# finleygou/GS-MARL

Measured on AMD Instinct MI355X. Metric: agent-steps/sec, coop-navigation 24 agents × 8192 envs, at 1/2/4/8 MI355X, higher is better.
Workload: dtype f32; 1 GPU; cooperative_navigation 24 agents x 8192 envs per GPU (24 goals, 24 obstacles; BASELINE headline / configs[4] shard); scenario=navigation, n_agents=24, n_envs_per_gpu=8192, global_envs=8192, episode_length=100, parallelism=env-sharded x1 (no data-path collective)

## Files before the change

gs-marl_amd/csrc/gsm_seg_kernels.hip:

```cpp
#include <type_traits>

#include "gsm_device.h"

namespace gsm {

template <typename T>
__device__ __forceinline__ T seg_scan(T v, int m) {
#pragma unroll
    for (int o = 1; o < kWave; o <<= 1) {
        const T u = __shfl_up(v, o);
        if (m >= o) v += u;
    }
    return v;
}

__device__ __forceinline__ int row_entity(int m, int N) { return m < N ? m : N + m; }

template <int kN, int kNo>
constexpr int envs_per_wave() {
    return kN > 0 ? ((kWave / (kN + kNo)) > kMaxSegEnvsPerWave ? kMaxSegEnvsPerWave : kWave / (kN + kNo))
                  : 0;
}

template <int kN, int kNo>
// ... 321 lines not shown
    }
    const uint32_t wb_lo = __builtin_amdgcn_readfirstlane((uint32_t)env_off);
    const uint32_t wb_hi = __builtin_amdgcn_readfirstlane((uint32_t)((uint64_t)env_off >> 32));
    const int64_t wbase = (int64_t)(((uint64_t)wb_hi << 32) | wb_lo);
    uint32_t o = (uint32_t)(env_off - wbase) + (uint32_t)(incl - c + (m >= N ? N : 0));
    const uint32_t goal_at = (uint32_t)(env_off - wbase) + (uint32_t)(a_total + m);
    if (!L.live || wbase >= out.cap) return;

    const float2 pm = s_pos[row_entity(m, N)];
    const uint32_t cap = (uint32_t)(out.cap - wbase);
    char *src = (char *)(out.index + wbase), *dst = (char *)(out.index + out.cap + wbase);
    char *attr = (char *)(out.attr + wbase);
    const int32_t g0 = (int32_t)(eb * E);
    const int32_t gs = g0 + row_entity(m, N);
    const uint64_t agent_bits = N >= 64 ? ~0ull : ((1ull << N) - 1);
    auto walk = [&](auto chk) {
        constexpr bool kChecked = decltype(chk)::value;
        auto put = [&](uint32_t at, int32_t a, int32_t b, float d) {
            if (!kChecked || at < cap) {
                const uint32_t byte = at << 2;
                *(int32_t *)(src + byte) = a;
                *(int32_t *)(dst + byte) = b;
                *(float *)(attr + byte) = d;
            }
        };
        auto edge_to = [&](int j, int32_t col) {
            const float2 q = s_pos[j];
            const float dx = pm.x - q.x, dy = pm.y - q.y;
            put(o++, gs, col, __builtin_amdgcn_sqrtf(dx * dx + dy * dy));
        };
        if constexpr (kG == 1 && kN > 0 && kN <= 32 && kN + kNo > 32) {
            const uint32_t gshift = L.agent ? 1u : 0u;
            if (L.agent) {
                const float2 q = s_pos[N + m];
                const float dx = pm.x - q.x, dy = pm.y - q.y;
                put(o + (uint32_t)__popcll(mask & agent_bits), gs, g0 + N + m,
                    __builtin_amdgcn_sqrtf(dx * dx + dy * dy));
            }
            uint64_t w = mask;
            while (w) {
                const int j = __builtin_ctzll(w);
                w &= w - 1;
                const bool ob = j >= kN;
                const int ent = ob ? kN + j : j;
                const float2 q = s_pos[ent];
                const float dx = pm.x - q.x, dy = pm.y - q.y;
                put(o + (ob ? gshift : 0u), gs, g0 + ent, __builtin_amdgcn_sqrtf(dx * dx + dy * dy));
                ++o;
            }
        } else if constexpr (kN > 0 && kN <= 32 && kNo <= 32) {
            uint32_t lo = (uint32_t)(mask & agent_bits), hi = (uint32_t)(mask >> kN);
            while (lo) {
                const int j = __builtin_ctz(lo);
                lo &= lo - 1;
                edge_to(j, g0 + j);
            }
            if (L.agent) edge_to(N + m, g0 + N + m);
            while (hi) {
                const int j = __builtin_ctz(hi);
                hi &= hi - 1;
                edge_to(2 * N + j, g0 + 2 * N + j);
            }
        } else {
            uint64_t lo = mask & agent_bits, hi = mask & ~agent_bits;
            while (lo) {
                const int j = __builtin_ctzll(lo);
                lo &= lo - 1;
                edge_to(j, g0 + j);
            }
            if (L.agent) edge_to(N + m, g0 + N + m);
            while (hi) {
                const int j = __builtin_ctzll(hi);
                hi &= hi - 1;
                edge_to(N + j, g0 + N + j);
            }
        }
        if (L.agent) {
            const float2 g = s_pos[N + m];
            const float dx = pm.x - g.x, dy = pm.y - g.y;
            put(goal_at, g0 + N + m, gs, __builtin_amdgcn_sqrtf(dx * dx + dy * dy));
        }
    };
    if (checked) walk(std::true_type{});
    else walk(std::false_type{});
}

template <int kN, int kNo>
__device__ __forceinline__ int stage_rows(const Lane &L, uint32_t *s_scr, int scr_cap, uint64_t mask, int incl) {
    constexpr int N = kN;
    static_assert(N <= 31 && kNo <= 32, "agent and obstacle column bits in one word each");
    const int m = L.m;
    const uint64_t mk = L.live ? mask : 0ull;
    const uint32_t lo = (uint32_t)mk & ((1u << N) - 1u), hi = (uint32_t)(mk >> N);
    const int c = __popc(lo) + __popc(hi) + (L.agent ? 1 : 0);
    const int a_total = __builtin_amdgcn_readlane(incl, N - 1);
    const int total = __builtin_amdgcn_readlane(incl, 63) + N;
    if (total > scr_cap) return -1;
    uint32_t *at = s_scr + (incl - c + (m >= N ? N : 0));
    const uint32_t src = (uint32_t)row_entity(m, N);
    for (uint32_t w = lo; w; w &= w - 1) *at++ = src | ((uint32_t)__builtin_ctz(w) << 8);
    if (L.agent) {
        *at++ = src | ((uint32_t)(N + m) << 8);
        s_scr[a_total + m] = (uint32_t)(N + m) | ((uint32_t)m << 8);
    }
    for (uint32_t w = hi; w; w &= w - 1) *at++ = src | ((uint32_t)(2 * N + __builtin_ctz(w)) << 8);
    wave_sync();
    return total;
}
template <int kN, int kNo>
__device__ __forceinline__ int stage_rows(const Lane &L, uint32_t *s_scr, int scr_cap, uint64_t mask) {
    const uint64_t mk = L.live ? mask : 0ull;
    const uint32_t lo = (uint32_t)mk & ((1u << kN) - 1u), hi = (uint32_t)(mk >> kN);
    const int c = __popc(lo) + __popc(hi) + (L.agent ? 1 : 0);
    return stage_rows<kN, kNo>(L, s_scr, scr_cap, mask, wave_scan(c));
}
template <int kN, int kNo>
__device__ __forceinline__ void write_staged(const Lane &L, const float2 *s_pos, const uint32_t *s_scr, int total,
                                             int64_t env_off, const EdgeSink &out) {
    constexpr int E = 2 * kN + kNo;
    const int64_t eb = L.b;
    const int32_t g0 = (int32_t)(eb * E);
    if (out.cap < ((int64_t)1 << 29)) {
        const uint32_t wb = (uint32_t)env_off, cap4 = (uint32_t)out.cap * 4u;
        char *const isrc = (char *)out.index, *const attr = (char *)out.attr;
        for (int e = L.lane; e < total; e += kWave) {
            const uint32_t w = s_scr[e];
            const uint32_t a = w & 0xffu, b = w >> 8;
            const float2 pa = s_pos[a], pb = s_pos[b];
            const float dx = pa.x - pb.x, dy = pa.y - pb.y;
            uint32_t byte = (wb + (uint32_t)e) << 2;
            asm("" : "+v"(byte));
            *(int32_t *)(isrc + byte) = g0 + (int32_t)a;
            *(int32_t *)(isrc + (byte + cap4)) = g0 + (int32_t)b;
            *(float *)(attr + byte) = __builtin_amdgcn_sqrtf(dx * dx + dy * dy);
        }
        return;
    }
    const uint32_t wb_lo = __builtin_amdgcn_readfirstlane((uint32_t)env_off);
    const uint32_t wb_hi = __builtin_amdgcn_readfirstlane((uint32_t)((uint64_t)env_off >> 32));
    const int64_t wbase = (int64_t)(((uint64_t)wb_hi << 32) | wb_lo);
    char *isrc = (char *)(out.index + wbase), *idst = (char *)(out.index + out.cap + wbase);
    char *attr = (char *)(out.attr + wbase);
    for (int e = L.lane; e < total; e += kWave) {
        const uint32_t w = s_scr[e];
        const uint32_t a = w & 0xffu, b = w >> 8;
        const float2 pa = s_pos[a], pb = s_pos[b];
        const float dx = pa.x - pb.x, dy = pa.y - pb.y;
        uint32_t byte = (uint32_t)e << 2;
        asm("" : "+v"(byte));
        *(int32_t *)(isrc + byte) = g0 + (int32_t)a;
        *(int32_t *)(idst + byte) = g0 + (int32_t)b;
        *(float *)(attr + byte) = __builtin_amdgcn_sqrtf(dx * dx + dy * dy);
    }
}

struct BlockPrefix {
    int cnt_k, acc;
};
__device__ __forceinline__ BlockPrefix block_prefix_loads(const int32_t *block_sum, const int32_t *edge_count,
                                                          int B, int G, const void *any16) {
    BlockPrefix r{0, 0};
    const int lane = threadIdx.x & 63, tid = threadIdx.x;
    const int first = blockIdx.x * kWavesPerBlock * G;
    const int nblk = min(kWavesPerBlock * G, B - first);
    const int ck = edge_count[first + min(lane, nblk - 1)];
    r.cnt_k = lane < nblk ? ck : 0;
    const int nb = (int)blockIdx.x, n4 = nb >> 2, nb4 = n4 << 2;
    const int4 *bs4 = n4 > 0 ? (const int4 *)block_sum : (const int4 *)any16;
    const int kc = n4 > 0 ? n4 - 1 : 0;
    const int4 q0 = bs4[min(tid, kc)], q1 = bs4[min(tid + kBlock, kc)];
    const int tl = block_sum[min(nb4 + tid, max(nb - 1, 0))];
    r.acc = (tid < n4 ? q0.x + q0.y + q0.z + q0.w : 0) + (tid + kBlock < n4 ? q1.x + q1.y + q1.z + q1.w : 0) +
            (tid < nb - nb4 ? tl : 0);
    for (int k = tid + 2 * kBlock; k < n4; k += kBlock) {
        const int4 q = bs4[k];
        r.acc += q.x + q.y + q.z + q.w;
    }
    return r;
}

template <int kN, int kNo, int kG>
__device__ __forceinline__ void block_emit(const DevParams &p, const Shape<kN, kNo> &s, const Lane &L,
                                           const float2 *s_pos, uint64_t mask, BlockPrefix pre, int *s_red,
                                           int64_t *edge_ptr, const EdgeSink &out, uint32_t *s_scr,
                                           int scr_cap) {
    const int first = blockIdx.x * kWavesPerBlock * s.G;
    constexpr bool kStaged = kG == 1 && kN > 0 && kN <= 31 && kNo <= 32;
    int staged = -1;
    if constexpr (kStaged) {
        if (L.b < p.B) staged = stage_rows<kN, kNo>(L, s_scr, scr_cap, mask);
    }
    const int acc = wave_total(pre.acc);
    const int incl_k = wave_scan(pre.cnt_k);
    if (L.lane == 0) s_red[L.wave] = acc;
    __syncthreads();
    int64_t base = 0;
    for (int q = 0; q < kWavesPerBlock; ++q) base += s_red[q];
    int my_cnt, before;
    if constexpr (kG == 1) {
        my_cnt = __builtin_amdgcn_readlane(pre.cnt_k, L.wave);
        before = __builtin_amdgcn_readlane(incl_k, L.wave) - my_cnt;
    } else {
        const int kk = L.live ? L.b - first : 0;
        my_cnt = __shfl(pre.cnt_k, kk);
        before = __shfl(incl_k, kk) - my_cnt;
    }
    const int64_t env_off = base + before;
    if (L.live && L.m == 0) {
        edge_ptr[L.b] = env_off;
        if (L.b == p.B - 1) edge_ptr[p.B] = env_off + my_cnt;
    }
    if constexpr (kStaged) {
        if (staged >= 0 && env_off + staged <= out.cap) {
            write_staged<kN, kNo>(L, s_pos, s_scr, staged, env_off, out);
            return;
        }
    }
    emit_rows<kN, kNo, kG>(s, L, s_pos, mask, env_off, out, env_off + my_cnt > out.cap);
}

struct SegIn {
    float2 x0, x1, v, u;
    uint64_t cand_prev, oo;
    int t, ep;
    float2 acc;
    float4 araw;
};

template <int kN, int kNo, int kFmt, bool kLag>
__device__ __forceinline__ SegIn seg_load(const DevParams &p, const Shape<kN, kNo> &s, const Lane &L) {
    static_assert(kN > 0 && kFmt >= 0, "compile-time shape and action format");
    constexpr int N = kN, E = 2 * kN + kNo, M = kN + kNo;
    SegIn in;
    const int64_t eb = L.b < p.B ? L.b : p.B - 1;
    const uint32_t lane = (uint32_t)L.lane;
    const uint32_t ma = lane < (uint32_t)N ? lane : N - 1, mm = lane < (uint32_t)M ? lane : M - 1;
    const float2 *pos_b = p.pos + eb * E;
    in.x0 = pos_b[lane < (uint32_t)E ? lane : E - 1];
    in.x1 = E > kWave ? pos_b[lane + kWave < (uint32_t)E ? lane + kWave : E - 1] : make_float2(0.0f, 0.0f);
    in.t = p.step_count[eb];
    in.ep = p.episode[eb];
    in.acc = p.ep_acc[eb];
    in.v = p.vel[eb * N + ma];
    const bool step = p.mode == kModeStep;
    const int64_t ai = eb * N + ma;
    if constexpr (kFmt == 0) {
        const float *q = (step ? (const float *)p.actions : p.node_feat) + ai * 5;
        in.araw = make_float4(q[1], q[2], q[3], q[4]);
    } else if constexpr (kFmt == 1) {
        const int32_t *q = step ? (const int32_t *)p.actions : (const int32_t *)p.node_feat;
        in.araw = make_float4(__int_as_float(q[ai]), 0.0f, 0.0f, 0.0f);
    } else {
        const float2 *q = step ? (const float2 *)p.actions : (const float2 *)p.node_feat;
        const float2 a = q[ai];
        in.araw = make_float4(a.x, a.y, 0.0f, 0.0f);
    }
    in.cand_prev = p.contact_mask[eb * N + ma];
    in.oo = p.row_mask[eb * M + mm];
    return in;
}

template <int kN, int kNo, int kFmt, bool kLag>
__device__ __forceinline__ void seg_load_finish(const DevParams &p, const Lane &L, SegIn &in) {
    const bool step = p.mode == kModeStep;
    const float4 a = in.araw;
    float ux, uy;
    if constexpr (kFmt == 0) {
        ux = a.x - a.y;
        uy = a.z - a.w;
    } else if constexpr (kFmt == 1) {
        const int k = __float_as_int(a.x);
        ux = (float)(k == 1) - (float)(k == 2);
        uy = (float)(k == 3) - (float)(k == 4);
    } else {
        ux = a.x;
        uy = a.y;
    }
    const bool ag_step = L.agent && step;
    in.u = ag_step ? make_float2(ux * p.sens, uy * p.sens) : make_float2(0.0f, 0.0f);
    in.cand_prev = ag_step ? in.cand_prev : 0ull;
    if (!L.agent) in.v = make_float2(0.0f, 0.0f);
    in.oo = (L.live && (kLag || L.m >= kN) && step) ? in.oo : 0ull;
    if (L.b >= p.B) {
        in.t = in.ep = 0;
        in.acc = make_float2(0.0f, 0.0f);
    }
}

template <int kN, int kNo, int kFmt, bool kLag>
__device__ __forceinline__ int seg_env(const DevParams &p, const Shape<kN, kNo> &s, const Lane &L,
                                       unsigned char *wave_lds, const SegIn &in, int64_t wid,
                                       BlockPrefix lag_pre, int *s_lag) {
    constexpr int kG = envs_per_wave<kN, kNo>();
    const int N = s.N, E = s.E, M = s.M, G = s.G;
    const int segc = L.seg < G ? L.seg : G - 1;
    float2 *s_pos = (float2 *)wave_lds + segc * E;
    float *s_nf = (float *)((float2 *)wave_lds + G * E);
    const int m = L.m;
    const bool obst = L.live && m >= N;
    const bool wave_live = kG == 1 ? L.b < p.B : true;
    const int64_t eb = kG == 1 ? (wave_live ? L.b : 0) : (L.live ? L.b : 0);
    const uint32_t um = (uint32_t)m;

    SegIn inf = in;
    if constexpr (kG == 1) seg_load_finish<kN, kNo, kFmt, kLag>(p, L, inf);
    int t = inf.t, ep = inf.ep;
// ... 596 lines not shown
            obs_sweep<kN, kNo, 1, kFused>(late_params(), s, L, s_pos, s_nf, pm2, true, 0ull, row2, cand2, cc2,
                                          coinc2, &Fn2, unext);
            if (reset) {
                pm = pm2;
                row = row2;
                cand = cand2;
                coinc = coinc2;
                Fn = Fn2;
            }
            if (!L.live) row = 0;
            scan = wave_scan(__popcll(row) + (L.agent ? 1 : 0));
            scan_tot = __builtin_amdgcn_readlane(scan, 63);
        }
        GSM_ACC(p, L.b, 15, tr0);
        const bool relaid = reset;
        if constexpr (kFused) {
            if (L.agent) s_force[m] = Fn;
        }

        KernargParams &q = late_params();
        const bool any_statics = (!kPlain && q.nf_full) || __any(relaid);
        if constexpr (kSlots) {
            if (L.live) {
                float *nf = q.ro.nf + k * q.ro.nf_s + eb * E * 7;
                if (L.agent) {
                    const float2 g = s_pos[N + m];
                    store_row(nf + m * 7, v, pm, make_float2(g.x - pm.x, g.y - pm.y), 0.0f);
                    if (any_statics)
                        store_row(nf + (N + m) * 7, make_float2(0.0f, 0.0f), g, make_float2(0.0f, 0.0f), 1.0f);
                } else if (any_statics) {
                    store_row(nf + (N + m) * 7, make_float2(0.0f, 0.0f), pm, make_float2(0.0f, 0.0f), 2.0f);
                }
            }
        } else {
            const uint32_t am = (uint32_t)((int)(um - (uint32_t)N) >> 31);
            const float2 g = s_pos[N + (um & am)];
            const float2 gr = make_float2(__uint_as_float(__float_as_uint(g.x - pm.x) & am),
                                          __uint_as_float(__float_as_uint(g.y - pm.y) & am));
            const float type = __uint_as_float(~am & 0x40000000u);
            char *nfb = (char *)q.ro.nf;
            const uint32_t env_el = (uint32_t)eb * (uint32_t)(E * 7);
            if (L.live && (L.agent || any_statics))
                store_row((float *)(nfb + (env_el + (um + (~am & (uint32_t)N)) * 7u) * 4u), v, pm, gr, type);
            if (L.agent && any_statics)
                store_row((float *)(nfb + (env_el + (um + (uint32_t)N) * 7u) * 4u), make_float2(0.0f, 0.0f), g,
                          make_float2(0.0f, 0.0f), 1.0f);
        }
        if (k == K - 1 && q.degenerate) {
            const uint64_t nb = __ballot(L.agent && nonfinite2(pm));
            deg = (uint8_t)((coinc ? kDegCoincident : 0) | (nb ? kDegNonfinite : 0));
        }
        const int wave_edges = (scan_tot & 0xffff) + (wave_live ? N : 0);
        if (wave_live && L.lane == 0) {
            (q.ro.done + (kSlots ? k * q.ro.done_s : 0))[L.b] = done ? 1 : 0;
            if (kSlots || k == K - 1) (q.ro.ecount + (kSlots ? k * q.ro.ec_s : 0))[L.b] = wave_edges;
        }

        GSM_REGION("publish");
        if (L.lane == 0) s_bc[r3 * kWavesPerBlock + wave] = wave_edges;
        GSM_ACC(p, L.b, 10, tw0);
        GSM_TNOW(tw1);
        __syncthreads();
        GSM_ACC(p, L.b, 11, tw1);
        if (threadIdx.x == 0) {
            int sum = 0;
            for (int w = 0; w < kWavesPerBlock; ++w) {
                s_pre[r3 * kWavesPerBlock + w] = sum;
                sum += s_bc[r3 * kWavesPerBlock + w];
            }
            const int cs = q.roll.csum_stride;
            prefix_publish(q.roll.gran + (int64_t)k * gridDim.x, csum_of(q) + (int64_t)k * nc * cs, cs,
                           (int)blockIdx.x, etag | (uint32_t)(k + 1), (uint32_t)sum);
            if (k == K - 1) {
                const int G = q.G, r = (int)blockIdx.x;
                if (G == 1) {
                    q.block_edge_sum[r] = sum;
                } else {
                    const int first = (r / G) * G, last = min(first + G, (int)gridDim.x) - 1;
                    if (r == last) {
                        const uint64_t *gk = q.roll.gran + (int64_t)k * gridDim.x;
                        const uint32_t tag = etag | (uint32_t)(k + 1);
                        int tot = sum;
                        for (int j = first; j < r; ++j) {
                            uint64_t x = gran_ld(gk + j);
                            if ((uint32_t)(x >> 32) != tag) x = roll_wait(gk + j, tag, q.roll.status);
                            tot += (int)(uint32_t)x;
                        }
                        q.block_edge_sum[r / G] = tot;
                    }
                }
            }
        }
        if (k == K - 1) GSM_RSTAMP(p, L.b, 4);
        if (k >= 2) emit_step(k - 2, r3n == 2 ? 0 : r3n + 1, r3n, s_row[L.lane], (int)s_inc[L.lane], pacing() ? k : 0, L);
        GSM_REGION("loop end");
        if (threadIdx.x == 0 && pacing())
            (void)__hip_atomic_fetch_add(pace_ctr(), 1u, __ATOMIC_RELAXED, __HIP_MEMORY_SCOPE_AGENT);
        if (k == 0) start_prio<1>();
        s_row[L.lane] = oo;
        s_inc[L.lane] = (uint32_t)inc_oo;
        oo = row;
        inc_oo = scan & 0xffff;
        cand_prev = L.agent ? cand : 0ull;
        const bool relaid_now = __any(relaid);
        if (__builtin_expect(relaid_now || relaid_prev, 0)) {
            float2 *const dst = pos_buf(r3n == 2 ? 0 : r3n + 1);
            for (int e = N + m; e < E; e += kWave) dst[e] = s_pos[e];
        }
        relaid_prev = relaid_now;
        if constexpr (!kFused) u = roll_force<kFmt>(late_params(), anext, L.agent);
        arow = nrow;
        r3 = r3n;
        wave_sync();
    }
    GSM_REGION("after the loop");
    KernargParams &q = late_params();
    if (wave_live) {
        float2 *const pos_b = q.pos + eb * E;
        const float2 *const s_pos = pos_buf(r3);
        const int n_rows = (kEager && !relaid_prev) ? N : E;
        if (L0.lane < n_rows) pos_b[L0.lane] = s_pos[L0.lane];
        if (L0.lane + kWave < n_rows) pos_b[L0.lane + kWave] = s_pos[L0.lane + kWave];
        if (L0.agent) {
            (q.vel + eb * N)[L0.lane] = v;
            (q.contact_mask + eb * N)[L0.lane] = cand_prev;
        }
        if (L0.live) (q.row_mask + eb * M)[L0.lane] = oo;
        if (L0.lane == 0) {
            q.step_count[L0.b] = t;
            q.episode[L0.b] = ep;
            q.ep_acc[L0.b] = acc;
            if (q.degenerate) q.degenerate[L0.b] = deg;
        }
    }
    {
        Lane L = L0;
        asm volatile("" : "+v"(L.lane), "+v"(L.m));
        GSM_RSTAMP(p, L.b, 5);
        const int rm1 = r3 == 0 ? 2 : r3 - 1;
        if (K >= 2) {
            __syncthreads();
            emit_step(K - 2, rm1, rm1 == 0 ? 2 : rm1 - 1, s_row[L.lane], (int)s_inc[L.lane], 0, L);
        }
        GSM_RSTAMP(p, L.b, 6);
        __syncthreads();
        emit_step(K - 1, r3, rm1, oo, inc_oo, 0, L);
        GSM_RSTAMP(p, L.b, 7);
    }
    GSM_RSTAMP(p, L0.b, 8);
}

#define GSM_PAIR_ATTR __attribute__((amdgpu_waves_per_eu(4, 4)))
constexpr int kPairHalf = 32, kPairEnvs = 2 * kWavesPerBlock;
constexpr int pair_lds_env(int N, int No, int E) { return roll_lds_force(E) + 8 * N + 8 * No; }
constexpr int pair_lds_wave(int N, int No, int E) { return 2 * pair_lds_env(N, No, E) + (8 + 8 + 4) * kWave; }
constexpr int pair_lds_block(int N, int No, int E) {
    return kWavesPerBlock * pair_lds_wave(N, No, E) + 4 * (6 * kPairEnvs + 4);
}

__device__ __forceinline__ int half_scan(int v) {
    v += dpp_i<0x111>(v);
    v += dpp_i<0x112>(v);
    v += dpp_i<0x114>(v);
    v += dpp_i<0x118>(v);
    v += dpp_i<0x142, 0xa>(v);
    return v;
}
__device__ __forceinline__ int half_sum_last(int v) {
    v += dpp_i<0xB1>(v);
    v += dpp_i<0x4E>(v);
    v += dpp_i<0x141>(v);
    v += dpp_i<0x140>(v);
    v += dpp_i<0x142, 0xa>(v);
    return v;
}
__device__ __forceinline__ float half_sum_last(float v) {
    v += dpp_f<0xB1>(v);
    v += dpp_f<0x4E>(v);
    v += dpp_f<0x141>(v);
    v += dpp_f<0x140>(v);
    v += dpp_f<0x142, 0xa>(v);
    return v;
}
__device__ __forceinline__ int half_last(int v, int h) {
    const int a = __builtin_amdgcn_readlane(v, 31), b = __builtin_amdgcn_readlane(v, 63);
    return h ? b : a;
}

template <int kN, int kNo, int kFmt>
__global__ __launch_bounds__(kBlock) GSM_PAIR_ATTR void gsm_roll_pair_kernel(DevParams p) {
    typedef float f32x2 __attribute__((ext_vector_type(2)));
    constexpr int N = kN, No = kNo, M = kN + kNo, E = 2 * kN + kNo;
    static_assert(M > 32 && M <= 64 && N <= 31 && No <= 32 && N % 2 == 0 && No % 2 == 0 && kFmt >= 0,
                  "two envs per wave: agent and obstacle rows in 32 lanes, column pairs");
    static_assert(E <= 3 * kPairHalf, "an env's positions in three passes of its half");
    static_assert(N * (M + 1) < (1 << 16) && No * M < (1 << 16), "neither half of the scan word carries");
    constexpr uint32_t abits = (1u << N) - 1u;
    constexpr int kEnvLds = pair_lds_env(N, No, E), wstride = pair_lds_wave(N, No, E);
    constexpr int scr_cap = 7 * E;
    extern __shared__ __attribute__((aligned(16))) unsigned char smem[];
    const int wave = __builtin_amdgcn_readfirstlane(threadIdx.x >> 6);
    const int lane = threadIdx.x & 63, h = lane >> 5, li = lane & (kPairHalf - 1);
    const int wb = (blockIdx.x * kWavesPerBlock + wave) * 2;
    const int b = wb + h;
    const bool env_live = b < p.B;
    const bool agent = env_live && li < N, obrow = env_live && li < No;
    const int64_t eb = env_live ? b : p.B - 1;
    const uint32_t ma = li < N ? (uint32_t)li : N - 1, mo = li < No ? (uint32_t)li : No - 1;
    unsigned char *const wave_lds = smem + wave * wstride;
    unsigned char *const envl = wave_lds + h * kEnvLds;
    float2 *const s_buf0 = (float2 *)envl;
    auto pos_buf = [&](int j3) { return s_buf0 + j3 * E; };
    float *const s_scr = (float *)(envl + roll_lds_scr(E));
    float2 *const s_force = (float2 *)(envl + roll_lds_force(E));
    float *const s_oxy = (float *)(s_force + N);
    uint64_t *const s_rowa = (uint64_t *)(wave_lds + 2 * kEnvLds);
    uint64_t *const s_rowo = s_rowa + kWave;
    uint32_t *const s_inc = (uint32_t *)(s_rowo + kWave);
    int *const s_bc = (int *)(smem + kWavesPerBlock * wstride);
    int *const s_red = s_bc + 3 * kPairEnvs;
    int *const s_pre = s_red + 4;
    const int slot = wave * 2 + h;

    start_prio<3>();
    const uint32_t epoch = p.roll.epoch;
    auto pace_ctr = [] { return (gu32 *)hand_chk(late_params().roll.pace + pace_key()); };
    uint32_t pace_v = 0;
    const int nc = ((int)gridDim.x + kPrefixChunk - 1) / kPrefixChunk;
    {
        KernargParams &qz = late_params();
        const int cs = qz.roll.csum_stride, n = qz.roll.K * nc;
        uint64_t *const cz = qz.roll.csum_next;
        for (int i = blockIdx.x * kBlock + threadIdx.x; i < n; i += gridDim.x * kBlock)
            __hip_atomic_store((gu64 *)hand_chk(cz + (int64_t)i * cs), 0ull, __ATOMIC_RELAXED,
                               __HIP_MEMORY_SCOPE_AGENT);
        for (int i = blockIdx.x * kBlock + threadIdx.x; i < kPaceKeys; i += gridDim.x * kBlock)
            __hip_atomic_store((gu32 *)hand_chk(qz.roll.pace_next + i * kPaceStride), 0u, __ATOMIC_RELAXED,
                               __HIP_MEMORY_SCOPE_AGENT);
        if (threadIdx.x == 0)
            pace_v = __hip_atomic_fetch_add(pace_ctr(), kPaceArrive, __ATOMIC_RELAXED, __HIP_MEMORY_SCOPE_AGENT);
    }

    const int K = p.roll.K, n_act = p.roll.n_actions;
    int arow = p.roll.t_first % n_act;
    const float2 *const pos_g = p.pos + eb * E;
    const float2 x0 = pos_g[li], x1 = pos_g[li + kPairHalf];
    const float2 x2 = pos_g[li + 2 * kPairHalf < E ? li + 2 * kPairHalf : E - 1];
    int t = p.step_count[eb], ep = p.episode[eb];
    float2 acc = p.ep_acc[eb];
    float2 v = p.vel[eb * N + ma];
    uint64_t cand_prev = p.contact_mask[eb * N + ma];
    uint64_t oo_a = p.row_mask[eb * M + ma], oo_o = p.row_mask[eb * M + N + mo];
    const float4 a0 = roll_action_load<kN, kFmt>(p, arow, eb, ma);
    if (!agent) {
        v = make_float2(0.0f, 0.0f);
        cand_prev = 0ull;
        oo_a = 0ull;
    }
    if (!obrow) oo_o = 0ull;
    if (!env_live) {
        t = ep = 0;
        acc = make_float2(0.0f, 0.0f);
    }
    if (env_live) {
        s_buf0[li] = s_buf0[E + li] = s_buf0[2 * E + li] = x0;
        s_buf0[li + kPairHalf] = s_buf0[E + li + kPairHalf] = s_buf0[2 * E + li + kPairHalf] = x1;
        if (li + 2 * kPairHalf < E)
            s_buf0[li + 2 * kPairHalf] = s_buf0[E + li + 2 * kPairHalf] = s_buf0[2 * E + li + 2 * kPairHalf] = x2;
    }
    if (threadIdx.x == 0) s_red[2] = (int)(pace_v >> 24);
    wave_sync();
    start_prio<2>();
    auto stage_obstacles = [&](const float2 *sp) {
        if (li < No) {
            const float2 q = sp[2 * N + li];
            const int at = (li >> 1) * 4 + (li & 1);
            s_oxy[at] = q.x;
            s_oxy[at + 2] = q.y;
        }
    };
    stage_obstacles(s_buf0);
    if (agent) {
        KernargParams &pc = late_params();
        s_force[li] = contact_walk(pc, roll_force<kFmt>(pc, a0, true), s_buf0[li], cand_prev, N,
                                   [&](int c) { return s_buf0[row_entity(c, N)]; });
    }

    auto sweep = [&](const float2 *sp, float2 pm, bool full, uint64_t oo_in, float4 anext, uint64_t &rowa,
                     uint64_t &rowo, uint64_t &cand, int &ccnt, bool &coinc, float2 &Fn) {
        KernargParams &q = late_params();
        if (agent) {
            const int at = (li >> 1) * 4 + (li & 1);
            s_scr[at] = pm.x;
            s_scr[at + 2] = pm.y;
        }
        const float2 pcol = agent ? pm : make_float2(1.0e18f, 1.0e18f);
        const float R2 = q.R2, cut2_aa = q.cut2_aa, cut2_ao = q.cut2_ao;
        uint32_t ra = 0, na = 0, ro = 0, no = 0;
        uint32_t oa = 0;
        wave_sync();
        const f32x2 px = {pcol.x, pcol.x}, py = {pcol.y, pcol.y};
        auto pair_d2 = [&](float4 Q) {
            const f32x2 dx = px - (f32x2){Q.x, Q.y};
            const f32x2 dy = py - (f32x2){Q.z, Q.w};
            return dx * dx + dy * dy;
        };
        const float4 *const xy4 = (const float4 *)s_scr, *const oxy4 = (const float4 *)s_oxy;
#pragma unroll
        for (int g = 0; g < N / 2; ++g) {
            const f32x2 d2 = pair_d2(xy4[g]);
            ra = shl1_add_lane(ra, __ballot(d2.x <= R2));
            na = shl1_add_lane(na, __ballot(d2.x < cut2_aa));
            ra = shl1_add_lane(ra, __ballot(d2.y <= R2));
            na = shl1_add_lane(na, __ballot(d2.y < cut2_aa));
        }
        auto obstacle_column = [&](int o, float d2) {
            const uint64_t b_rad = __ballot(d2 <= R2);
            ro = shl1_add_lane(ro, b_rad);
            no = shl1_add_lane(no, __ballot(d2 < cut2_ao));
            oa = writelane_u32((uint32_t)b_rad, (uint32_t)o, oa);
            oa = writelane_u32((uint32_t)(b_rad >> 32), (uint32_t)(kPairHalf + o), oa);
        };
#pragma unroll
        for (int g = 0; g < No / 2; ++g) {
            const f32x2 d2 = pair_d2(oxy4[g]);
            obstacle_column(2 * g, d2.x);
            obstacle_column(2 * g + 1, d2.y);
        }
        ra = __builtin_bitreverse32(ra) >> (32 - N);
        na = __builtin_bitreverse32(na) >> (32 - N);
        ro = __builtin_bitreverse32(ro) >> (32 - No);
        no = __builtin_bitreverse32(no) >> (32 - No);
        uint64_t r = ((uint64_t)ro << N) | ra;
        const uint64_t near = ((uint64_t)no << N) | na;
        if (agent) r &= ~(1ull << li);
        else r = 0ull;
        uint64_t orow = (full ? 0ull : (oo_in & ~(uint64_t)abits)) | oa;
        if (full && obrow) {
            const float2 po = sp[2 * N + li];
#pragma unroll 2
            for (int k = 0; k < No; ++k) {
                const float2 qk = sp[2 * N + k];
                const float dx = po.x - qk.x, dy = po.y - qk.y;
                const float d2 = dx * dx + dy * dy;
                if (d2 > 0.0f && d2 <= R2) orow |= 1ull << (N + k);
            }
        }
        if (!obrow) orow = 0ull;
        int cc = 0;
        uint64_t c = 0;
        bool coincident = false;
        if (agent) {
            uint64_t w = near & ~(1ull << li);
            c = w;
            const float2 f0 = roll_force<kFmt>(q, anext, true);
            float Fx = f0.x, Fy = f0.y;
            const float dmin_aa = q.dmin_aa, dmin_ao = q.dmin_ao;
            while (w) {
                const int k = __builtin_ctzll(w);
                w &= w - 1;
                const float2 qk = sp[k < N ? k : N + k];
                const float dx = pm.x - qk.x, dy = pm.y - qk.y;
                const float d2 = dx * dx + dy * dy;
                cc += d2 < (k < N ? q.dmin2_aa : q.dmin2_ao) ? 1 : 0;
                if (d2 == 0.0f) {
                    c &= ~(1ull << k);
                    coincident = true;
                } else {
                    const float f = contact_scale(q, d2, k < N ? dmin_aa : dmin_ao);
                    Fx += f * dx;
                    Fy += f * dy;
                }
            }
            Fn = make_float2(Fx, Fy);
        }
        const uint64_t cb = __ballot(coincident);
        coinc = (h ? (uint32_t)(cb >> 32) : (uint32_t)cb) != 0u;
        if (__builtin_expect(cb != 0ull, 0)) {
            if (coinc && agent) {
                uint64_t ex = 0;
#pragma unroll 1
                for (int k = 0; k < M; ++k) {
                    const float2 qk = sp[k < N ? k : N + k];
                    const float dx = pm.x - qk.x, dy = pm.y - qk.y;
                    const float d2 = dx * dx + dy * dy;
                    if (d2 > 0.0f && d2 <= R2) ex |= 1ull << k;
                }
                r = ex;
            }
            if (coinc && obrow) {
                const float2 po = sp[2 * N + li];
                uint64_t ex = 0;
#pragma unroll 1
                for (int k = 0; k < N; ++k) {
                    const float2 qk = sp[k];
                    const float dx = po.x - qk.x, dy = po.y - qk.y;
                    const float d2 = dx * dx + dy * dy;
                    if (d2 > 0.0f && d2 <= R2) ex |= 1ull << k;
                }
                orow = (orow & ~(uint64_t)abits) | ex;
            }
        }
        rowa = r;
        rowo = orow;
        cand = c;
        ccnt = cc;
    };
    auto list_word = [&](uint64_t rowa, uint64_t rowo) {
        return (agent ? __popcll(rowa) + 1 : 0) | (__popcll(rowo) << 16);
    };

    const uint32_t etag = roll_epoch_tag(epoch);
    uint8_t deg = 0;
    auto emit_step = [&](const int j, const int pj3, const int cj3, const uint64_t rowa, const uint64_t rowo,
                         const int inc, const int steps_done) {
        GSM_REGION("staging");
        const int tot = half_last(inc, h);
        const int a_total = tot & 0xffff, total = a_total + N + (tot >> 16);
        int staged = -1;
        if (env_live && total <= scr_cap) {
            uint32_t *const scr = (uint32_t *)s_scr;
            const uint32_t lo = (uint32_t)rowa & abits, hi = (uint32_t)(rowa >> N);
            if (agent) {
                uint32_t *at = scr + ((inc & 0xffff) - (__popc(lo) + __popc(hi) + 1));
                const uint32_t src = (uint32_t)li;
                for (uint32_t w = lo; w; w &= w - 1) *at++ = src | ((uint32_t)__builtin_ctz(w) << 8);
                *at++ = src | ((uint32_t)(N + li) << 8);
                scr[a_total + li] = (uint32_t)(N + li) | ((uint32_t)li << 8);
                for (uint32_t w = hi; w; w &= w - 1) *at++ = src | ((uint32_t)(2 * N + __builtin_ctz(w)) << 8);
            }
            if (obrow) {
                const uint32_t olo = (uint32_t)rowo & abits, ohi = (uint32_t)(rowo >> N);
                uint32_t *at = scr + (a_total + N + (inc >> 16) - (__popc(olo) + __popc(ohi)));
                const uint32_t src = (uint32_t)(2 * N + li);
                for (uint32_t w = olo; w; w &= w - 1) *at++ = src | ((uint32_t)__builtin_ctz(w) << 8);
                for (uint32_t w = ohi; w; w &= w - 1) *at++ = src | ((uint32_t)(2 * N + __builtin_ctz(w)) << 8);
            }
            staged = total;
        }
        wave_sync();
        GSM_REGION("prefix");
        if (wave == 0) {
            KernargParams &qe = late_params();
            const uint32_t pv =
                steps_done > 0 ? __hip_atomic_load(pace_ctr(), __ATOMIC_RELAXED, __HIP_MEMORY_SCOPE_AGENT) : 0u;
            const int cs = qe.roll.csum_stride;
            const int ex = roll_prefix(qe.roll.gran + (int64_t)j * gridDim.x, qe.roll.csum + (int64_t)j * nc * cs, cs,
                                       etag | (uint32_t)(j + 1), qe.roll.status, lane);
            const int lvl = steps_done > 0 ? pace_level((uint32_t)__builtin_amdgcn_readfirstlane(pv), steps_done,
                                                        __builtin_amdgcn_readfirstlane(s_red[2]), qe.roll.pace_q)
                                           : 1;
            if (lane == 0) {
                s_red[0] = ex;
                s_red[1] = lvl;
            }
        }
        __syncthreads();
        GSM_REGION("write");
        if (steps_done > 0) pace_set(__builtin_amdgcn_readfirstlane(s_red[1]));
        const int before = s_pre[cj3 * kPairEnvs + slot];
        const int my_cnt = s_bc[cj3 * kPairEnvs + slot];
        int64_t env_off = (int64_t)s_red[0] + before;
        KernargParams &qs = late_params();
        if (env_off < 0) {
            if (li == 0)
                __hip_atomic_store((gu32 *)qs.roll.status, 2u, __ATOMIC_RELAXED, __HIP_MEMORY_SCOPE_AGENT);
            env_off = qs.ro.cap;
        }
        if (env_live && li == 0) {
            qs.ro.eptr[b] = env_off;
            if (b == qs.B - 1) qs.ro.eptr[qs.B] = env_off + my_cnt;
        }
        const EdgeSink out = roll_edge_sink<false>(qs, j, K);
#pragma unroll
        for (int hh = 0; hh < 2; ++hh) {
            if (wb + hh >= qs.B) break;
            const int st = __builtin_amdgcn_readlane(staged, hh * kPairHalf);
            const uint32_t off_lo = __builtin_amdgcn_readlane((uint32_t)env_off, hh * kPairHalf);
            const uint32_t off_hi = __builtin_amdgcn_readlane((uint32_t)((uint64_t)env_off >> 32), hh * kPairHalf);
            const int64_t off = (int64_t)(((uint64_t)off_hi << 32) | off_lo);
            const float2 *const s_prev = (const float2 *)(wave_lds + hh * kEnvLds) + pj3 * E;
            if (st >= 0 && off + st <= out.cap) {
                Lane Lw{};
                Lw.lane = lane;
                Lw.b = wb + hh;
                write_staged<kN, kNo>(Lw, s_prev, (const uint32_t *)(wave_lds + hh * kEnvLds + roll_lds_scr(E)), st, off,
                                      out);
            } else if (h == hh) {
                const int32_t g0 = (int32_t)((int64_t)b * E);
                auto put = [&](int64_t at, int32_t a, int32_t d) {
                    if (at < out.cap) {
                        const float2 pa = s_prev[a], pd = s_prev[d];
                        const float dx = pa.x - pd.x, dy = pa.y - pd.y;
                        out.index[at] = g0 + a;
                        out.index[out.cap + at] = g0 + d;
                        out.attr[at] = __builtin_amdgcn_sqrtf(dx * dx + dy * dy);
                    }
                };
                if (agent) {
                    const uint32_t lo = (uint32_t)rowa & abits, hi = (uint32_t)(rowa >> N);
                    int64_t o = off + ((inc & 0xffff) - (__popc(lo) + __popc(hi) + 1));
                    for (uint32_t w = lo; w; w &= w - 1) put(o++, li, __builtin_ctz(w));
                    put(o++, li, N + li);
                    for (uint32_t w = hi; w; w &= w - 1) put(o++, li, 2 * N + __builtin_ctz(w));
                    put(off + a_total + li, N + li, li);
                }
                if (obrow) {
                    const uint32_t olo = (uint32_t)rowo & abits, ohi = (uint32_t)(rowo >> N);
                    int64_t o = off + a_total + N + ((inc >> 16) - (__popc(olo) + __popc(ohi)));
                    for (uint32_t w = olo; w; w &= w - 1) put(o++, 2 * N + li, __builtin_ctz(w));
                    for (uint32_t w = ohi; w; w &= w - 1) put(o++, 2 * N + li, 2 * N + __builtin_ctz(w));
                }
            }
        }
        wave_sync();
    };

    GSM_REGION("before the loop");
    int r3 = 0;
    int inc_oo = 0;
    bool relaid_prev = false;
    for (int k = 0; k < K; ++k) {
        GSM_REGION("integration");
        const int nrow = arow + 1 == n_act ? 0 : arow + 1;
        const float4 anext = roll_action_load<kN, kFmt>(late_params(), nrow, eb, ma);
        const int r3n = r3 == 2 ? 0 : r3 + 1;
        const float2 *const s_cur = pos_buf(r3);
        float2 *const s_pos = pos_buf(r3n);
        KernargParams &pc = late_params();
        if (agent) {
            const float2 pi = s_cur[li];
            const float2 F = s_force[li];
            s_pos[li] = integrate_agent(pc, v, pi, F.x, F.y, 0.0f);
        }
        wave_sync();
        t += 1;
        const bool done = env_live && t >= pc.EL;

        GSM_REGION("sweep");
        float2 pm = s_pos[ma];
        uint64_t rowa, rowo, cand;
        int ccnt;
        bool coinc;
        float2 Fn = make_float2(0.0f, 0.0f);
        sweep(s_pos, pm, false, oo_o, anext, rowa, rowo, cand, ccnt, coinc, Fn);

        GSM_REGION("reward and stores");
        float r = 0.0f;
        if (agent) {
            const float2 g = s_pos[N + li];
            const float dx = pm.x - g.x, dy = pm.y - g.y;
            r = -__builtin_amdgcn_sqrtf(dx * dx + dy * dy);
        }
        const float rs = half_sum_last(r);
        const float rs_a = __int_as_float(__builtin_amdgcn_readlane(__float_as_int(rs), 31));
        const float rs_b = __int_as_float(__builtin_amdgcn_readlane(__float_as_int(rs), 63));
        const float rsum = h ? rs_b : rs_a;
        const int ci = agent ? ccnt : 0;
        const int csum = half_last(half_sum_last(ci), h);
        int scan = half_scan(list_word(rowa, rowo));
        if (agent) {
            KernargParams &q = late_params();
            const uint32_t off = ((uint32_t)eb * (uint32_t)N + (uint32_t)li) * 4u;
            *(float *)((char *)q.ro.rew + off) = r;
            *(float *)((char *)q.ro.cost + off) = (float)ci;
        }
        if (env_live) {
            acc.x += rsum;
            acc.y += (float)csum;
        }
        const bool reset = done;
        if (reset && li == 0) late_params().ep_last[b] = acc;
        if (__any(reset)) {
            if (reset) {
                ep = ep + 1;
                t = 0;
                acc = make_float2(0.0f, 0.0f);
                v = make_float2(0.0f, 0.0f);
                const uint32_t gid = (uint32_t)(late_params().env_base + b);
                for (int e = li; e < E; e += kPairHalf) s_pos[e] = layout_pos(p, gid, (uint32_t)ep, (uint32_t)e);
            }
            wave_sync();
            stage_obstacles(s_pos);
            const float2 pm2 = s_pos[ma];
            uint64_t rowa2, rowo2, cand2;
            int cc2;
            bool coinc2;
            float2 Fn2 = make_float2(0.0f, 0.0f);
            sweep(s_pos, pm2, true, 0ull, anext, rowa2, rowo2, cand2, cc2, coinc2, Fn2);
            if (reset) {
                pm = pm2;
                rowa = rowa2;
                rowo = rowo2;
                cand = cand2;
                coinc = coinc2;
                Fn = Fn2;
            }
            scan = half_scan(list_word(rowa, rowo));
        }
        const bool relaid = reset;
        if (agent) s_force[li] = Fn;

        KernargParams &q = late_params();
        {
            float *const nf = q.ro.nf + eb * (E * 7);
            if (agent) {
                const float2 g = s_pos[N + li];
                store_row(nf + li * 7, v, pm, make_float2(g.x - pm.x, g.y - pm.y), 0.0f);
                if (relaid) store_row(nf + (N + li) * 7, make_float2(0.0f, 0.0f), g, make_float2(0.0f, 0.0f), 1.0f);
            }
            if (obrow && relaid)
                store_row(nf + (2 * N + li) * 7, make_float2(0.0f, 0.0f), s_pos[2 * N + li], make_float2(0.0f, 0.0f),
                          2.0f);
        }
        if (k == K - 1 && q.degenerate) {
            const uint64_t nb = __ballot(agent && nonfinite2(pm));
            const bool nfh = (h ? (uint32_t)(nb >> 32) : (uint32_t)nb) != 0u;
            deg = (uint8_t)((coinc ? kDegCoincident : 0) | (nfh ? kDegNonfinite : 0));
        }
        const int tot = half_last(scan, h);
        const int env_edges = (tot & 0xffff) + (tot >> 16) + (env_live ? N : 0);
        if (env_live && li == 0) {
            q.ro.done[b] = done ? 1 : 0;
            if (k == K - 1) q.ro.ecount[b] = env_edges;
        }

        GSM_REGION("publish");
        if (li == 0) s_bc[r3 * kPairEnvs + slot] = env_edges;
        __syncthreads();
        if (threadIdx.x == 0) {
            int sum = 0, first4 = 0;
            for (int w = 0; w < kPairEnvs; ++w) {
                if (w == kWavesPerBlock) first4 = sum;
                s_pre[r3 * kPairEnvs + w] = sum;
                sum += s_bc[r3 * kPairEnvs + w];
            }
            const int cs = q.roll.csum_stride;
            prefix_publish(q.roll.gran + (int64_t)k * gridDim.x, q.roll.csum + (int64_t)k * nc * cs, cs,
                           (int)blockIdx.x, etag | (uint32_t)(k + 1), (uint32_t)sum);
            if (k == K - 1) {
                const int rb = (int)blockIdx.x;
                q.block_edge_sum[2 * rb] = first4;
                if ((2 * rb + 1) * kWavesPerBlock < q.B) q.block_edge_sum[2 * rb + 1] = sum - first4;
            }
        }
        if (k >= 2) emit_step(k - 2, r3n == 2 ? 0 : r3n + 1, r3n, s_rowa[lane], s_rowo[lane], (int)s_inc[lane], k);
        GSM_REGION("loop end");
        if (threadIdx.x == 0)
            (void)__hip_atomic_fetch_add(pace_ctr(), 1u, __ATOMIC_RELAXED, __HIP_MEMORY_SCOPE_AGENT);
        if (k == 0) start_prio<1>();
        s_rowa[lane] = oo_a;
        s_rowo[lane] = oo_o;
        s_inc[lane] = (uint32_t)inc_oo;
        oo_a = rowa;
        oo_o = rowo;
        inc_oo = scan;
        cand_prev = agent ? cand : 0ull;
        const bool relaid_now = __any(relaid);
        if (__builtin_expect(relaid_now || relaid_prev, 0)) {
            float2 *const dst = pos_buf(r3n == 2 ? 0 : r3n + 1);
            for (int e = N + li; e < E; e += kPairHalf) dst[e] = s_pos[e];
        }
// ... 703 lines not shown
```

Baseline: 33.55 billion agent-steps/s.

## Stage both paired envs' edges into one shared list and write them together

Reorganizes the pair kernel's LDS so both half-wave envs share interleaved position buffers and a single staging area. Each staged word now carries an output-offset delta in its upper bits. Both envs' edges are then emitted in one pass through a new write_staged_pair helper instead of two serialized per-env passes, and goal edges are written directly rather than staged. This is meant to cut wasted lane work and loop overhead in the edge write phase, at the cost of more complex packing, an 8-bit entity limit across both envs, and a fallback path when an env's list does not fit.

```diff
diff --git a/gs-marl_amd/csrc/gsm_seg_kernels.hip b/gs-marl_amd/csrc/gsm_seg_kernels.hip
--- a/gs-marl_amd/csrc/gsm_seg_kernels.hip
+++ b/gs-marl_amd/csrc/gsm_seg_kernels.hip
@@ -497,6 +497,33 @@
         *(int32_t *)(idst + byte) = g0 + (int32_t)b;
         *(float *)(attr + byte) = __builtin_amdgcn_sqrtf(dx * dx + dy * dy);
     }
+}
+
+template <int kN>
+__device__ __forceinline__ void write_staged_pair(int lane, const float2 *s_pos, const uint32_t *s_scr, int total,
+                                                  int64_t base, int32_t g0, bool goal, int64_t goal_at,
+                                                  uint32_t gent, const EdgeSink &out) {
+    auto lists = [&](char *isrc, char *idst, char *attr, uint32_t wb) {
+        auto put = [&](uint32_t at, uint32_t a, uint32_t b) {
+            const float2 pa = s_pos[a], pb = s_pos[b];
+            const float dx = pa.x - pb.x, dy = pa.y - pb.y;
+            uint32_t byte = at << 2;
+            asm("" : "+v"(byte));
+            *(int32_t *)(isrc + byte) = g0 + (int32_t)a;
+            *(int32_t *)(idst + byte) = g0 + (int32_t)b;
+            *(float *)(attr + byte) = __builtin_amdgcn_sqrtf(dx * dx + dy * dy);
+        };
+        if (goal) put(wb + (uint32_t)(goal_at - base), gent, gent - (uint32_t)kN);
+        for (int e = lane; e < total; e += kWave) {
+            const uint32_t w = s_scr[e];
+            put(wb + (uint32_t)e + (w >> 16), w & 0xffu, (w >> 8) & 0xffu);
+        }
+    };
+    if (out.cap < ((int64_t)1 << 29)) {
+        lists((char *)out.index, (char *)(out.index + out.cap), (char *)out.attr, (uint32_t)base);
+        return;
+    }
+    lists((char *)(out.index + base), (char *)(out.index + out.cap + base), (char *)(out.attr + base), 0u);
 }
 
 struct BlockPrefix {
@@ -1399,8 +1426,12 @@
 
 #define GSM_PAIR_ATTR __attribute__((amdgpu_waves_per_eu(4, 4)))
 constexpr int kPairHalf = 32, kPairEnvs = 2 * kWavesPerBlock;
-constexpr int pair_lds_env(int N, int No, int E) { return roll_lds_force(E) + 8 * N + 8 * No; }
-constexpr int pair_lds_wave(int N, int No, int E) { return 2 * pair_lds_env(N, No, E) + (8 + 8 + 4) * kWave; }
+constexpr int pair_lds_scr(int E) { return (3 * 2 * 8 * E + 15) & ~15; }
+constexpr int pair_lds_env(int E) { return (28 * E + 15) & ~15; }
+constexpr int pair_lds_force(int E) { return pair_lds_scr(E) + 2 * pair_lds_env(E); }
+constexpr int pair_lds_wave(int N, int No, int E) {
+    return pair_lds_force(E) + 2 * (8 * N + 8 * No) + (8 + 8 + 4) * kWave;
+}
 constexpr int pair_lds_block(int N, int No, int E) {
     return kWavesPerBlock * pair_lds_wave(N, No, E) + 4 * (6 * kPairEnvs + 4);
 }
@@ -1443,8 +1474,9 @@
     static_assert(E <= 3 * kPairHalf, "an env's positions in three passes of its half");
     static_assert(N * (M + 1) < (1 << 16) && No * M < (1 << 16), "neither half of the scan word carries");
     constexpr uint32_t abits = (1u << N) - 1u;
-    constexpr int kEnvLds = pair_lds_env(N, No, E), wstride = pair_lds_wave(N, No, E);
-    constexpr int scr_cap = 7 * E;
+    static_assert(2 * E <= 256, "both envs' entities in the 8-bit fields of a staged word");
+    constexpr int wstride = pair_lds_wave(N, No, E);
+    constexpr int scr_cap = 7 * E - N;
     extern __shared__ __attribute__((aligned(16))) unsigned char smem[];
     const int wave = __builtin_amdgcn_readfirstlane(threadIdx.x >> 6);
     const int lane = threadIdx.x & 63, h = lane >> 5, li = lane & (kPairHalf - 1);
@@ -1455,13 +1487,13 @@
     const int64_t eb = env_live ? b : p.B - 1;
     const uint32_t ma = li < N ? (uint32_t)li : N - 1, mo = li < No ? (uint32_t)li : No - 1;
     unsigned char *const wave_lds = smem + wave * wstride;
-    unsigned char *const envl = wave_lds + h * kEnvLds;
-    float2 *const s_buf0 = (float2 *)envl;
-    auto pos_buf = [&](int j3) { return s_buf0 + j3 * E; };
-    float *const s_scr = (float *)(envl + roll_lds_scr(E));
-    float2 *const s_force = (float2 *)(envl + roll_lds_force(E));
-    float *const s_oxy = (float *)(s_force + N);
-    uint64_t *const s_rowa = (uint64_t *)(wave_lds + 2 * kEnvLds);
+    float2 *const s_buf0 = (float2 *)wave_lds + h * E;
+    auto pos_buf = [&](int j3) { return s_buf0 + j3 * (2 * E); };
+    uint32_t *const s_stage = (uint32_t *)(wave_lds + pair_lds_scr(E));
+    float *const s_scr = (float *)(wave_lds + pair_lds_scr(E) + h * pair_lds_env(E));
+    float2 *const s_force = (float2 *)(wave_lds + pair_lds_force(E)) + h * N;
+    float *const s_oxy = (float *)(wave_lds + pair_lds_force(E) + 2 * 8 * N) + h * (2 * No);
+    uint64_t *const s_rowa = (uint64_t *)(wave_lds + pair_lds_force(E) + 2 * (8 * N + 8 * No));
     uint64_t *const s_rowo = s_rowa + kWave;
     uint32_t *const s_inc = (uint32_t *)(s_rowo + kWave);
     int *const s_bc = (int *)(smem + kWavesPerBlock * wstride);
@@ -1510,10 +1542,10 @@
         acc = make_float2(0.0f, 0.0f);
     }
     if (env_live) {
-        s_buf0[li] = s_buf0[E + li] = s_buf0[2 * E + li] = x0;
-        s_buf0[li + kPairHalf] = s_buf0[E + li + kPairHalf] = s_buf0[2 * E + li + kPairHalf] = x1;
-        if (li + 2 * kPairHalf < E)
-            s_buf0[li + 2 * kPairHalf] = s_buf0[E + li + 2 * kPairHalf] = s_buf0[2 * E + li + 2 * kPairHalf] = x2;
+        float2 *const b1 = pos_buf(1), *const b2 = pos_buf(2);
+        s_buf0[li] = b1[li] = b2[li] = x0;
+        s_buf0[li + kPairHalf] = b1[li + kPairHalf] = b2[li + kPairHalf] = x1;
+        if (li + 2 * kPairHalf < E) s_buf0[li + 2 * kPairHalf] = b1[li + 2 * kPairHalf] = b2[li + 2 * kPairHalf] = x2;
     }
     if (threadIdx.x == 0) s_red[2] = (int)(pace_v >> 24);
     wave_sync();
@@ -1662,28 +1694,30 @@
     auto emit_step = [&](const int j, const int pj3, const int cj3, const uint64_t rowa, const uint64_t rowo,
                          const int inc, const int steps_done) {
         GSM_REGION("staging");
-        const int tot = half_last(inc, h);
-        const int a_total = tot & 0xffff, total = a_total + N + (tot >> 16);
-        int staged = -1;
-        if (env_live && total <= scr_cap) {
-            uint32_t *const scr = (uint32_t *)s_scr;
-            const uint32_t lo = (uint32_t)rowa & abits, hi = (uint32_t)(rowa >> N);
+        const int tot_a = __builtin_amdgcn_readlane(inc, kPairHalf - 1), tot_b = __builtin_amdgcn_readlane(inc, kWave - 1);
+        const int st_a = (tot_a & 0xffff) + (tot_a >> 16), st_b = (tot_b & 0xffff) + (tot_b >> 16);
+        const bool fit_a = st_a <= scr_cap, fit_b = st_b <= scr_cap;
+        const int in_a = fit_a ? st_a : 0, staged = in_a + (fit_b ? st_b : 0);
+        const int a_total = (h ? tot_b : tot_a) & 0xffff;
+        const bool fits = h ? fit_b : fit_a;
+        if (fits) {
+            const uint32_t ent = (uint32_t)(h * E) * 0x101u;
+            uint32_t *const scr = s_stage + (h ? in_a : 0);
             if (agent) {
+                const uint32_t lo = (uint32_t)rowa & abits, hi = (uint32_t)(rowa >> N);
                 uint32_t *at = scr + ((inc & 0xffff) - (__popc(lo) + __popc(hi) + 1));
-                const uint32_t src = (uint32_t)li;
-                for (uint32_t w = lo; w; w &= w - 1) *at++ = src | ((uint32_t)__builtin_ctz(w) << 8);
-                *at++ = src | ((uint32_t)(N + li) << 8);
-                scr[a_total + li] = (uint32_t)(N + li) | ((uint32_t)li << 8);
-                for (uint32_t w = hi; w; w &= w - 1) *at++ = src | ((uint32_t)(2 * N + __builtin_ctz(w)) << 8);
+                const uint32_t src = ent + (uint32_t)li + ((uint32_t)(h * N) << 16);
+                for (uint32_t w = lo; w; w &= w - 1) *at++ = src + ((uint32_t)__builtin_ctz(w) << 8);
+                *at++ = src + ((uint32_t)(N + li) << 8);
+                for (uint32_t w = hi; w; w &= w - 1) *at++ = src + ((uint32_t)(2 * N + __builtin_ctz(w)) << 8);
             }
             if (obrow) {
                 const uint32_t olo = (uint32_t)rowo & abits, ohi = (uint32_t)(rowo >> N);
-                uint32_t *at = scr + (a_total + N + (inc >> 16) - (__popc(olo) + __popc(ohi)));
-                const uint32_t src = (uint32_t)(2 * N + li);
-                for (uint32_t w = olo; w; w &= w - 1) *at++ = src | ((uint32_t)__builtin_ctz(w) << 8);
-                for (uint32_t w = ohi; w; w &= w - 1) *at++ = src | ((uint32_t)(2 * N + __builtin_ctz(w)) << 8);
-            }
-            staged = total;
+                uint32_t *at = scr + (a_total + (inc >> 16) - (__popc(olo) + __popc(ohi)));
+                const uint32_t src = ent + (uint32_t)(2 * N + li) + ((uint32_t)((h + 1) * N) << 16);
+                for (uint32_t w = olo; w; w &= w - 1) *at++ = src + ((uint32_t)__builtin_ctz(w) << 8);
+                for (uint32_t w = ohi; w; w &= w - 1) *at++ = src + ((uint32_t)(2 * N + __builtin_ctz(w)) << 8);
+            }
         }
         wave_sync();
         GSM_REGION("prefix");
@@ -1719,25 +1753,22 @@
             if (b == qs.B - 1) qs.ro.eptr[qs.B] = env_off + my_cnt;
         }
         const EdgeSink out = roll_edge_sink<false>(qs, j, K);
-#pragma unroll
-        for (int hh = 0; hh < 2; ++hh) {
-            if (wb + hh >= qs.B) break;
-            const int st = __builtin_amdgcn_readlane(staged, hh * kPairHalf);
-            const uint32_t off_lo = __builtin_amdgcn_readlane((uint32_t)env_off, hh * kPairHalf);
-            const uint32_t off_hi = __builtin_amdgcn_readlane((uint32_t)((uint64_t)env_off >> 32), hh * kPairHalf);
-            const int64_t off = (int64_t)(((uint64_t)off_hi << 32) | off_lo);
-            const float2 *const s_prev = (const float2 *)(wave_lds + hh * kEnvLds) + pj3 * E;
-            if (st >= 0 && off + st <= out.cap) {
-                Lane Lw{};
-                Lw.lane = lane;
-                Lw.b = wb + hh;
-                write_staged<kN, kNo>(Lw, s_prev, (const uint32_t *)(wave_lds + hh * kEnvLds + roll_lds_scr(E)), st, off,
-                                      out);
-            } else if (h == hh) {
+        if (wb < qs.B) {
+            const uint32_t off_lo = __builtin_amdgcn_readlane((uint32_t)env_off, 0);
+            const uint32_t off_hi = __builtin_amdgcn_readlane((uint32_t)((uint64_t)env_off >> 32), 0);
+            const int64_t off_a = (int64_t)(((uint64_t)off_hi << 32) | off_lo);
+            const int edges = st_a + N + (wb + 1 < qs.B ? st_b + N : 0);
+            const bool in_range = off_a + edges <= out.cap;
+            const float2 *const s_prev = (const float2 *)wave_lds + pj3 * (2 * E);
+            if (in_range)
+                write_staged_pair<kN>(lane, s_prev, s_stage, staged, off_a + (st_a - in_a), (int32_t)((int64_t)wb * E),
+                                      agent && fits, env_off + a_total + li, (uint32_t)(h * E + N + li), out);
+            if (env_live && !(in_range && fits)) {
+                const float2 *const s_own = s_prev + h * E;
                 const int32_t g0 = (int32_t)((int64_t)b * E);
                 auto put = [&](int64_t at, int32_t a, int32_t d) {
                     if (at < out.cap) {
-                        const float2 pa = s_prev[a], pd = s_prev[d];
+                        const float2 pa = s_own[a], pd = s_own[d];
                         const float dx = pa.x - pd.x, dy = pa.y - pd.y;
                         out.index[at] = g0 + a;
                         out.index[out.cap + at] = g0 + d;
@@ -1746,15 +1777,15 @@
                 };
                 if (agent) {
                     const uint32_t lo = (uint32_t)rowa & abits, hi = (uint32_t)(rowa >> N);
-                    int64_t o = off + ((inc & 0xffff) - (__popc(lo) + __popc(hi) + 1));
+                    int64_t o = env_off + ((inc & 0xffff) - (__popc(lo) + __popc(hi) + 1));
                     for (uint32_t w = lo; w; w &= w - 1) put(o++, li, __builtin_ctz(w));
                     put(o++, li, N + li);
                     for (uint32_t w = hi; w; w &= w - 1) put(o++, li, 2 * N + __builtin_ctz(w));
-                    put(off + a_total + li, N + li, li);
+                    put(env_off + a_total + li, N + li, li);
                 }
                 if (obrow) {
                     const uint32_t olo = (uint32_t)rowo & abits, ohi = (uint32_t)(rowo >> N);
-                    int64_t o = off + a_total + N + ((inc >> 16) - (__popc(olo) + __popc(ohi)));
+                    int64_t o = env_off + a_total + N + ((inc >> 16) - (__popc(olo) + __popc(ohi)));
                     for (uint32_t w = olo; w; w &= w - 1) put(o++, 2 * N + li, __builtin_ctz(w));
                     for (uint32_t w = ohi; w; w &= w - 1) put(o++, 2 * N + li, 2 * N + __builtin_ctz(w));
                 }
```

Result: faster. 35.29 billion agent-steps/s (median of 6 runs) (+5.2%).
